# Tencent/PocketFlow

Hardware: NVIDIA H100
Metric: images_per_sec_compression_aware_training_step (higher is better)
Workload: dtype f32

## Files before the change

### pocketflow_b200/csrc/pf_conv_tma.cu

```cuda
#include <cuda.h>

#include "pf_conv_tc.cuh"
#include "pf_tma.cuh"

namespace pfconv {
using namespace pftma;

constexpr int kTmaMaxStages = 8;
constexpr int kTmaThreads = (kMmaWarps + 1) * 32;

struct TmaP {
  int M, Ng, BN, nk, n_tiles, total_tiles;
  int cblocks, R, S;
  int rows_hw, rows_w;
  int src_h, src_w;
  int base_w, base_h, str_w, str_h, flip;
  int na, nb;
  int accumulate, relu, ring, stage_budget;
  int chunked;
  FastDiv d_hw, d_w, d_ntiles, d_cblocks, d_s;
  EpiAff aff;
  const pf_tc_act_hdr* a_hdr;
  const float* csum;
  int nseg;
  pf_tc_bn_out bn;
};

constexpr int kPingPongWarps = 4;
constexpr int kPingPongThreads = (kMmaWarps + 4) * 32;
constexpr int kProducerRegs = 40, kConsumerRegs = 232;

__device__ __forceinline__ void conv_tma_epilogue_chunked(float (&acc)[2][64], const TmaP& p, float* acc_s,
                                                          int n0, long long off, long long* rowoff, float* out,
                                                          const float* bias, int wg, int q, int lane) {
  constexpr int P = acc_pitch(32);
  float* r0 = acc_s + (size_t)(16 * q + (lane >> 2)) * P + 2 * (lane & 3);
#pragma unroll
  for (int ch = 0; ch < 4; ++ch) {
    if (ch > 0) named_bar_sync(2 + wg, 128);
#pragma unroll
    for (int h = 0; h < 2; ++h)
#pragma unroll
      for (int jj = 0; jj < 4; ++jj) {
        const int j = 4 * ch + jj;
        *reinterpret_cast<float2*>(r0 + (size_t)(64 * h) * P + 8 * jj) = make_float2(acc[h][4 * j], acc[h][4 * j + 1]);
        *reinterpret_cast<float2*>(r0 + (size_t)(64 * h + 8) * P + 8 * jj) =
            make_float2(acc[h][4 * j + 2], acc[h][4 * j + 3]);
      }
    named_bar_sync(2 + wg, 128);
    epilogue_rows<0>(acc_s + (size_t)(32 * q) * P, 0, 32, off, rowoff, out, nullptr, bias, p.relu, n0 + 32 * ch, 32,
                     p.Ng, lane, nullptr, p.aff, 0.f, nullptr, nullptr, 0, p.bn);
  }
}

template <int AFF, int BN, int NA, int NB, bool BNO, bool U8>
__device__ __forceinline__ void conv_tma_consumer(const TmaP& p, uint8_t* smem, uint32_t stage_bytes,
                                                  uint32_t n_stages, uint64_t* full_bar, uint64_t* empty_bar,
                                                  uint64_t* ml_bar, uint64_t* epi_bar, int* tab_n0, float* out,
                                                  const float* bias, const float* residual) {
  const int tid = threadIdx.x, warp = tid >> 5, lane = tid & 31;
  const int wg = warp >> 2, q = warp & 3, wtid = tid & 127;
  constexpr uint32_t kRow = U8 ? 64u : 128u, kATile = TM * kRow;
  const uint32_t b_bytes = (uint32_t)BN * kRow;
  float* acc_s = reinterpret_cast<float*>(smem + p.stage_budget);
  long long* rowoff_all = reinterpret_cast<long long*>(acc_s + TM * acc_pitch(p.chunked ? 32 : BN));
  float* jrow_all = reinterpret_cast<float*>(rowoff_all + kMmaWarps * 32);
  float* aff_tab = jrow_all + kMmaWarps * 32;
  uint8_t* ring_all = reinterpret_cast<uint8_t*>(aff_tab + (AFF == 2 ? 2 * 256 : 0) + (BNO ? 4 * kMaxBN : 0));
  long long* rowoff = rowoff_all + warp * 32;
  float* jrow = jrow_all + warp * 32;
  uint8_t* ring = p.ring ? ring_all + (size_t)warp * p.ring * kRingSlotBytes : nullptr;
  const float* extra = residual ? residual : (p.accumulate ? out : nullptr);
  uint32_t it = (uint32_t)wg * (uint32_t)p.nk;
  for (int tile = blockIdx.x + wg * gridDim.x, j = 0; tile < p.total_tiles; tile += 2 * gridDim.x, ++j) {
    const bool wait_turn = wg == 1 || j > 0;
    const uint32_t turn_ph = (uint32_t)(wg == 1 ? j : j - 1) & 1u;
    if (wait_turn) mbar_wait_bounded(&ml_bar[wg], turn_ph);
    std::conditional_t<U8, int, float> acc[2][BN / 2];
#pragma unroll
    for (int h = 0; h < 2; ++h)
#pragma unroll
      for (int i = 0; i < BN / 2; ++i) acc[h][i] = 0;
    uint32_t s = it % n_stages, ph = (it / n_stages) & 1u, prev = 0;
    for (int ks = 0; ks < p.nk; ++ks) {
      mbar_wait_bounded(&full_bar[s], ph);
      const uint32_t a0 = smem_u32(smem + (size_t)s * stage_bytes), a1 = a0 + kATile;
      const uint32_t b0 = a0 + (uint32_t)NA * kATile, b1 = b0 + b_bytes;
      wgmma_fence();
      if constexpr (U8) {
#pragma unroll
        for (int kk = 0; kk < 2; ++kk) {
          const uint64_t db = make_smem_desc(b0 + kk * 32, 16, 512, kSwizzle64B);
#pragma unroll
          for (int h = 0; h < 2; ++h)
            WgmmaU8<BN>::mma(acc[h], make_smem_desc(a0 + (uint32_t)h * 64 * 64 + kk * 32, 16, 512, kSwizzle64B), db);
        }
      } else {
#pragma unroll
        for (int kk = 0; kk < BK / 16; ++kk) {
          const uint64_t db0 = make_smem_desc(b0 + kk * 32, 16, 1024), db1 = make_smem_desc(b1 + kk * 32, 16, 1024);
#pragma unroll
          for (int h = 0; h < 2; ++h) {
            const uint32_t ha = (uint32_t)h * 64 * 128 + kk * 32;
            wg_mma_kslice<BN, 0, NA, NB>(acc[h], make_smem_desc(a0 + ha, 16, 1024), make_smem_desc(a1 + ha, 16, 1024),
                                         db0, db1);
          }
        }
      }
      wgmma_commit();
      wgmma_wait<1>(acc);
      if (ks > 0) {
        __syncwarp();
        if (lane == 0) mbar_arrive(&empty_bar[prev]);
      }
      prev = s;
      if (++s == n_stages) { s = 0; ph ^= 1u; }
    }
    __syncwarp();
    if (lane == 0) mbar_arrive(&ml_bar[wg ^ 1]);
    wgmma_wait<0>(acc);
    if (p.nk > 0) {
      __syncwarp();
      if (lane == 0) mbar_arrive(&empty_bar[prev]);
    }
    it += 2u * (uint32_t)p.nk;
    const int mt = (int)fdiv((uint32_t)tile, p.d_ntiles);
    const int n0 = (tile - mt * p.n_tiles) * BN;
    const int m = mt * TM + q * 32 + lane;
    const long long off = m < p.M ? (long long)m * p.Ng : -1;
    float my_j = 0.f;
    if (AFF == 2 && p.csum && m < p.M) {
      const int img = (int)fdiv((uint32_t)m, p.d_hw);
      const int rem = m - img * p.rows_hw;
      const int y = (int)fdiv((uint32_t)rem, p.d_w), x = rem - y * p.rows_w;
      const int ow0 = p.base_w + x * p.str_w, oh0 = p.base_h + y * p.str_h;
      const int total = p.R * p.S * p.nseg;
      const float* cbase = p.csum + (size_t)img * p.src_h * p.src_w * p.nseg;
      auto term = [&](int u) -> float {
        if (u >= total) return 0.f;
        const int t = u / p.nseg, g = u - t * p.nseg;
        const int r = (int)fdiv((uint32_t)t, p.d_s), s_ = t - r * p.S;
        const int ih = oh0 + r, iw = ow0 + s_;
        const bool ok = (unsigned)ih < (unsigned)p.src_h && (unsigned)iw < (unsigned)p.src_w;
        return ok ? __ldg(cbase + ((size_t)ih * p.src_w + iw) * p.nseg + g) : 0.f;
      };
      float a0 = 0.f, a1 = 0.f, a2 = 0.f, a3 = 0.f;
      for (int u = 0; u < total; u += 4) {
        const float v0 = term(u), v1 = term(u + 1), v2 = term(u + 2), v3 = term(u + 3);
        a0 += v0; a1 += v1; a2 += v2; a3 += v3;
      }
      my_j = (a0 + a1) + (a2 + a3);
    }
    if (wait_turn) mbar_wait_bounded(&epi_bar[wg], turn_ph);
    constexpr bool TAB = AFF == 2 || BNO;
    if constexpr (BN == 128 && AFF == 0 && !BNO && !U8) {
      if (p.chunked) {
        conv_tma_epilogue_chunked(acc, p, acc_s, n0, off, rowoff, out, bias, wg, q, lane);
        __syncwarp();
        if (lane == 0) mbar_arrive(&epi_bar[wg ^ 1]);
        continue;
      }
    }
    wgmma_store_acc<BN>(acc[0], acc_s, acc_pitch(BN), 0, wtid);
    wgmma_store_acc<BN>(acc[1], acc_s, acc_pitch(BN), 64, wtid);
    const int tab_was = TAB ? *reinterpret_cast<volatile int*>(tab_n0) : 0;
    if (AFF == 2 && tab_was != n0) {
      float a_s = p.aff.a_scale ? __ldg(p.aff.a_scale) : 1.f;
      if (U8 && __ldg(&p.a_hdr->nplanes) != 1) a_s = __int_as_float(0x7fc00000);
      for (int c = wtid; c < BN; c += 128) {
        const bool cok = n0 + c < p.Ng;
        const int bi = p.aff.per_channel ? n0 + c : 0;
        const float al = cok ? __ldg(p.aff.w_alpha + bi) : 0.f, be = cok ? __ldg(p.aff.w_beta + bi) : 0.f;
        const float sx = al * p.aff.w_rk;
        aff_tab[c] = sx * a_s;
        aff_tab[256 + c] = fmaf(p.aff.w_centre, sx, be) * a_s;
      }
    }
    if (BNO && tab_was != n0) bn_table(p.bn, aff_tab + (AFF == 2 ? 512 : 0), n0, BN, p.Ng, wtid, 128);
    named_bar_sync(2 + wg, 128);
    if (TAB && tab_was != n0 && wtid == 0) *reinterpret_cast<volatile int*>(tab_n0) = n0;
    epilogue_rows<AFF, BNO>(acc_s + (size_t)(32 * q) * acc_pitch(BN), 0, 32, off, rowoff, out, extra, bias, p.relu, n0,
                            BN, p.Ng, lane, ring, p.aff, my_j, jrow, TAB ? aff_tab : nullptr, p.ring, p.bn);
    __syncwarp();
    if (lane == 0) mbar_arrive(&epi_bar[wg ^ 1]);
  }
}

template <int AFF, int BN, bool BNO = false, bool U8 = false>
__global__ void __launch_bounds__(kPingPongThreads, 1)
conv_tma_kernel(const __grid_constant__ CUtensorMap tmA0, const __grid_constant__ CUtensorMap tmA1,
                const __grid_constant__ CUtensorMap tmB0, const __grid_constant__ CUtensorMap tmB1,
                float* __restrict__ out, const float* __restrict__ bias, const float* __restrict__ residual,
                const __grid_constant__ TmaP p) {
  extern __shared__ uint8_t smem_raw[];
  uint8_t* smem = (uint8_t*)(((uintptr_t)smem_raw + 1023) & ~(uintptr_t)1023);
  __shared__ uint64_t full_bar[kTmaMaxStages], empty_bar[kTmaMaxStages], ml_bar[2], epi_bar[2];
  __shared__ int tab_n0;
  const int tid = threadIdx.x, warp = tid >> 5, lane = tid & 31;
  int na = p.na;
  if (p.a_hdr) na = (__ldg(&p.a_hdr->nplanes) == 2) ? 2 : 1;
  const int nb = p.nb;
  constexpr uint32_t kRow = U8 ? 64u : 128u, kATile = TM * kRow;
  const uint32_t b_bytes = (uint32_t)BN * kRow;
  const uint32_t stage_bytes = (uint32_t)na * kATile + (uint32_t)nb * b_bytes;
  const uint32_t n_stages = min((uint32_t)kTmaMaxStages, (uint32_t)p.stage_budget / stage_bytes);

  if (tid == 0) {
    for (int s = 0; s < kTmaMaxStages; ++s) {
      mbar_init(&full_bar[s], 1);
      mbar_init(&empty_bar[s], kPingPongWarps);
    }
    for (int w = 0; w < 2; ++w) {
      mbar_init(&ml_bar[w], kPingPongWarps);
      mbar_init(&epi_bar[w], kPingPongWarps);
    }
    tab_n0 = -1;
    fence_barrier_init();
  }
  __syncthreads();

  if (warp >= kMmaWarps) {
    setmaxnreg_dec<kProducerRegs>();
    if (warp == kMmaWarps && lane == 0) {
      prefetch_map(&tmA0);
      prefetch_map(&tmB0);
      if (na == 2) prefetch_map(&tmA1);
      if (nb == 2) prefetch_map(&tmB1);
      uint32_t s = 0, ph = 0;
      for (int tile = blockIdx.x; tile < p.total_tiles; tile += gridDim.x) {
        const int mt = (int)fdiv((uint32_t)tile, p.d_ntiles);
        const int n0 = (tile - mt * p.n_tiles) * BN;
        const int m0 = mt * TM;
        const int img = (int)fdiv((uint32_t)m0, p.d_hw);
        const int rem = m0 - img * p.rows_hw;
        const int y = (int)fdiv((uint32_t)rem, p.d_w), x = rem - y * p.rows_w;
        const int cw = p.base_w + x * p.str_w, ch = p.base_h + y * p.str_h;
        for (int ks = 0; ks < p.nk; ++ks) {
          mbar_wait_bounded(&empty_bar[s], ph ^ 1u);
          const int tap = (int)fdiv((uint32_t)ks, p.d_cblocks);
          const int cb = ks - tap * p.cblocks;
          const int r = (int)fdiv((uint32_t)tap, p.d_s), q = tap - r * p.S;
          const uint32_t ow = (uint32_t)(p.flip ? p.S - 1 - q : q), oh = (uint32_t)(p.flip ? p.R - 1 - r : r);
          const uint32_t sa = smem_u32(smem + (size_t)s * stage_bytes);
          const uint32_t sb = sa + (uint32_t)na * kATile;
          mbar_arrive_expect_tx(&full_bar[s], stage_bytes);
          load_im2col(sa, &tmA0, &full_bar[s], cb * BK, cw, ch, img, ow, oh);
          if (na == 2) load_im2col(sa + kATile, &tmA1, &full_bar[s], cb * BK, cw, ch, img, ow, oh);
          load_2d(sb, &tmB0, &full_bar[s], ks * BK, n0);
          if (nb == 2) load_2d(sb + b_bytes, &tmB1, &full_bar[s], ks * BK, n0);
          if (++s == n_stages) { s = 0; ph ^= 1u; }
        }
      }
    }
  } else {
    setmaxnreg_inc<kConsumerRegs>();
#define PF_TMA_CONSUMER(NA_, NB_)                                                                                    \
  conv_tma_consumer<AFF, BN, NA_, NB_, BNO, U8>(p, smem, stage_bytes, n_stages, full_bar, empty_bar, ml_bar, epi_bar, \
                                                &tab_n0, out, bias, residual)
    if constexpr (U8) {
      PF_TMA_CONSUMER(1, 1);
    } else {
      if (na == 2) {
        if (nb == 2) PF_TMA_CONSUMER(2, 2);
        else PF_TMA_CONSUMER(2, 1);
      } else {
        if (nb == 2) PF_TMA_CONSUMER(1, 2);
        else PF_TMA_CONSUMER(1, 1);
      }
    }
#undef PF_TMA_CONSUMER
  }
}

struct WgTmaP {
  TcGeom g;
  int Mtot, Npix, pps, splits, BN, n_tiles, tiles, total_units;
  int na, nb, stage_budget;
  FastDiv d_pq, d_q, d_c, d_s, d_tiles, d_ntiles;
  EpiAff aff;
  const pf_tc_act_hdr* x_hdr;
};
constexpr uint32_t kWgBlockBytes = BK * 128;

template <int AFF, int BN>
__global__ void __launch_bounds__(kTmaThreads, 1)
conv_tma_wgrad_kernel(const __grid_constant__ CUtensorMap tmX0, const __grid_constant__ CUtensorMap tmX1,
                      const __grid_constant__ CUtensorMap tmY0, const __grid_constant__ CUtensorMap tmY1,
                      float* __restrict__ partial, const __grid_constant__ WgTmaP p) {
  extern __shared__ uint8_t smem_raw[];
  uint8_t* smem = (uint8_t*)(((uintptr_t)smem_raw + 1023) & ~(uintptr_t)1023);
  __shared__ uint64_t full_bar[kTmaMaxStages], empty_bar[kTmaMaxStages];
  const int tid = threadIdx.x, warp = tid >> 5, lane = tid & 31;
  const TcGeom& g = p.g;
  const int nblkB = BN / 64;
  int na = p.na;
  if (p.x_hdr) na = (__ldg(&p.x_hdr->nplanes) == 2) ? 2 : 1;
  const int nb = p.nb;
  const uint32_t a_bytes = 2 * kWgBlockBytes, b_bytes = (uint32_t)nblkB * kWgBlockBytes;
  const uint32_t stage_bytes = (uint32_t)na * a_bytes + (uint32_t)nb * b_bytes;
  const uint32_t n_stages = min((uint32_t)kTmaMaxStages, (uint32_t)p.stage_budget / stage_bytes);
  float* acc_s = reinterpret_cast<float*>(smem + p.stage_budget);
  long long* rowoff_all = reinterpret_cast<long long*>(acc_s + TM * acc_pitch(BN));
  float* jrow_all = reinterpret_cast<float*>(rowoff_all + kMmaWarps * 32);
  if (tid == 0) {
    for (int s = 0; s < kTmaMaxStages; ++s) {
      mbar_init(&full_bar[s], 1);
      mbar_init(&empty_bar[s], kMmaWarps);
    }
    fence_barrier_init();
  }
  __syncthreads();
  struct Unit {
    int split, m0, n0, pbeg, nk;
  };
  auto decode = [&](int u) -> Unit {
    Unit r;
    r.split = (int)fdiv((uint32_t)u, p.d_tiles);
    const int t = u - r.split * p.tiles;
    const int mt = (int)fdiv((uint32_t)t, p.d_ntiles);
    r.m0 = mt * TM;
    r.n0 = (t - mt * p.n_tiles) * BN;
    r.pbeg = r.split * p.pps;
    const int pend = min(p.Npix, r.pbeg + p.pps);
    r.nk = (pend - r.pbeg + BK - 1) / BK;
    return r;
  };

  if (warp == kMmaWarps) {
    if (lane == 0) {
      prefetch_map(&tmX0);
      prefetch_map(&tmY0);
      if (na == 2) prefetch_map(&tmX1);
      if (nb == 2) prefetch_map(&tmY1);
      const int pq = g.P * g.Q;
      uint32_t s = 0, ph = 0;
      for (int u = blockIdx.x; u < p.total_units; u += gridDim.x) {
        const Unit un = decode(u);
        int c0[2], tr[2], tq[2], nvalid = 0;
#pragma unroll
        for (int b = 0; b < 2; ++b) {
          const int kf = un.m0 + 64 * b;
          const int tap = (int)fdiv((uint32_t)kf, p.d_c);
          c0[b] = kf - tap * g.C;
          tr[b] = (int)fdiv((uint32_t)tap, p.d_s);
          tq[b] = tap - tr[b] * g.S;
          if (kf < p.Mtot) nvalid = b + 1;
        }
        const uint32_t tx = (uint32_t)na * (uint32_t)nvalid * kWgBlockBytes + (uint32_t)nb * b_bytes;
        for (int ks = 0; ks < un.nk; ++ks) {
          mbar_wait_bounded(&empty_bar[s], ph ^ 1u);
          const int pix0 = un.pbeg + ks * BK;
          const int pn = (int)fdiv((uint32_t)pix0, p.d_pq);
          const int rem = pix0 - pn * pq;
          const int oh = (int)fdiv((uint32_t)rem, p.d_q), ow = rem - oh * g.Q;
          const int cw = ow * g.sw - g.pl, ch = oh * g.sh - g.pt;
          const uint32_t sa = smem_u32(smem + (size_t)s * stage_bytes);
          const uint32_t sb = sa + (uint32_t)na * a_bytes;
          mbar_arrive_expect_tx(&full_bar[s], tx);
          for (int b = 0; b < nvalid; ++b) {
            load_im2col(sa + b * kWgBlockBytes, &tmX0, &full_bar[s], c0[b], cw, ch, pn, (uint32_t)tq[b], (uint32_t)tr[b]);
            if (na == 2)
              load_im2col(sa + a_bytes + b * kWgBlockBytes, &tmX1, &full_bar[s], c0[b], cw, ch, pn, (uint32_t)tq[b],
                          (uint32_t)tr[b]);
          }
          for (int j = 0; j < nblkB; ++j) {
            load_2d(sb + j * kWgBlockBytes, &tmY0, &full_bar[s], un.n0 + 64 * j, pix0);
            if (nb == 2) load_2d(sb + b_bytes + j * kWgBlockBytes, &tmY1, &full_bar[s], un.n0 + 64 * j, pix0);
          }
          if (++s == n_stages) { s = 0; ph ^= 1u; }
        }
      }
    }
  } else {
    const int wg = warp >> 2, q = warp & 3;
    long long* rowoff = rowoff_all + warp * 32;
    float* jrow = jrow_all + warp * 32;
    auto consume = [&](auto na_c, auto nb_c) {
    constexpr int NA = decltype(na_c)::value, NB = decltype(nb_c)::value;
    uint32_t s = 0, ph = 0;
    for (int u = blockIdx.x; u < p.total_units; u += gridDim.x) {
      const Unit un = decode(u);
      float acc[BN / 2];
#pragma unroll
      for (int i = 0; i < BN / 2; ++i) acc[i] = 0.f;
      uint32_t prev = 0;
      for (int ks = 0; ks < un.nk; ++ks) {
        mbar_wait_bounded(&full_bar[s], ph);
        const uint32_t base = smem_u32(smem + (size_t)s * stage_bytes);
        const uint32_t a0 = base + (uint32_t)wg * kWgBlockBytes, a1 = a0 + a_bytes;
        const uint32_t b0 = base + (uint32_t)NA * a_bytes, b1 = b0 + b_bytes;
        wg_mma_stage<BN, 1, NA, NB>(acc, a0, a1, b0, b1, 2048, 2048, kWgBlockBytes, 1024, kWgBlockBytes, 1024);
        wgmma_wait<1>(acc);
        if (ks > 0) {
          __syncwarp();
          if (lane == 0) mbar_arrive(&empty_bar[prev]);
        }
        prev = s;
        if (++s == n_stages) { s = 0; ph ^= 1u; }
      }
      wgmma_wait<0>(acc);
      if (un.nk > 0) {
        __syncwarp();
        if (lane == 0) mbar_arrive(&empty_bar[prev]);
      }
      const int em = un.m0 + q * 32 + lane;
      const long long off = em < p.Mtot ? ((long long)un.split * p.Mtot + em) * g.K : -1;
      wg_tile_to_smem<BN>(acc, acc_s, tid);
      epilogue_tile_a<AFF>(acc_s, warp, off, rowoff, partial, nullptr, nullptr, 0, un.n0, BN, g.K, lane, nullptr, p.aff,
                           0.f, jrow, pf_tc_bn_out{});
    }
    };
    using one = std::integral_constant<int, 1>;
    using two = std::integral_constant<int, 2>;
    if (na == 2) {
      if (nb == 2) consume(two(), two());
      else consume(two(), one());
    } else {
      if (nb == 2) consume(one(), two());
      else consume(one(), one());
    }
  }
}

static int g_feed_override = -1;
void conv_tma_set_feed(int mode) { g_feed_override = mode < 0 ? -1 : (mode ? 1 : 0); }
static bool tma_enabled() {
  if (g_feed_override >= 0) return g_feed_override == 1;
  static int on = -1;
  if (on < 0) {
    const char* v = getenv("PF_TC_FEED");
    on = !(v && strcmp(v, "lsu") == 0);
  }
  return on == 1;
}

bool conv_tma_eligible(int pass, const TcGeom& g) {
  if (!tma_enabled()) return false;
  if (pass == 0) return g.C % 64 == 0 && g.K % 16 == 0 && g.sh <= 8 && g.sw <= 8 && g.R <= 16 && g.S <= 16;
  if (pass == 1) return g.K % 64 == 0 && g.C % 16 == 0 && g.sh == 1 && g.sw == 1 && g.R <= 16 && g.S <= 16;
  return g.C % 64 == 0 && g.K % 64 == 0 && g.sh <= 8 && g.sw <= 8;
}

bool conv_tma_u8_eligible(const TcGeom& g) {
  return g.C % 64 == 0 && g.K % 64 == 0 && g.sh <= 8 && g.sw <= 8 && g.R <= 16 && g.S <= 16;
}

static int pick_bn(int Ng) {
  int BN = Ng >= 128 ? 128 : (Ng >= 64 ? 64 : (Ng >= 32 ? 32 : 16));
  const int forced = env_int("PF_TC_BN", 0);
  if (forced >= 16 && forced <= kMaxBN && forced <= ((Ng + 15) / 16) * 16 && (forced & (forced - 1)) == 0) BN = forced;
  return BN;
}

#define PF_TMA_ENCODE(call, who)                                                               \
  do {                                                                                         \
    const int e__ = (call);                                                                    \
    if (e__ != 0) {                                                                            \
      pf_set_error("%s: tensor-map encoding failed (%d): %s", who, e__, #call);                \
      return PF_ERR_INVALID_ARG;                                                               \
    }                                                                                          \
  } while (0)

int conv_tma_launch(int pass, const TcGeom& g, const pf_tc_act& a, const pf_tc_wt& w, float* out, int accumulate,
                    const float* bias, int relu, const float* residual, cudaStream_t st, const char* who,
                    const pf_tc_bn_out* bn, bool u8) {
  TmaP p;
  memset(&p, 0, sizeof(p));
  const int CC = pass == 0 ? g.C : g.K;
  const int Hs = pass == 0 ? g.H : g.P, Ws = pass == 0 ? g.W : g.Q;
  const int Ho = pass == 0 ? g.P : g.H, Wo = pass == 0 ? g.Q : g.W;
  const int64_t M64 = (int64_t)g.N * Ho * Wo;
  PF_REQUIRE(M64 < (1ll << 31), "%s: too many rows", who);
  p.M = (int)M64;
  p.Ng = pass == 0 ? g.K : g.C;
  const int Kdim = g.R * g.S * CC;
  p.nk = Kdim / BK;
  p.cblocks = CC / BK;
  p.R = g.R;
  p.S = g.S;
  p.rows_hw = Ho * Wo;
  p.rows_w = Wo;
  p.src_h = Hs;
  p.src_w = Ws;
  if (pass == 0) {
    p.base_w = -g.pl; p.base_h = -g.pt; p.str_w = g.sw; p.str_h = g.sh; p.flip = 0;
  } else {
    p.base_w = g.pl - (g.S - 1); p.base_h = g.pt - (g.R - 1); p.str_w = 1; p.str_h = 1; p.flip = 1;
  }
  p.accumulate = accumulate;
  p.relu = relu;
  const int m_tiles = (p.M + TM - 1) / TM;
  const int BN = u8 ? (p.Ng >= 128 ? 128 : 64) : pick_bn(p.Ng);
  p.BN = BN;
  p.n_tiles = (p.Ng + BN - 1) / BN;
  p.total_tiles = m_tiles * p.n_tiles;
  p.d_hw = make_fastdiv((uint32_t)p.rows_hw);
  p.d_w = make_fastdiv((uint32_t)p.rows_w);
  p.d_ntiles = make_fastdiv((uint32_t)p.n_tiles);
  p.d_cblocks = make_fastdiv((uint32_t)p.cblocks);
  p.d_s = make_fastdiv((uint32_t)g.S);
  p.na = a.plane1 ? 2 : 1;
  p.nb = w.plane1 ? 2 : 1;
  p.a_hdr = a.hdr;
  PF_REQUIRE(a.hdr == nullptr || a.plane1 != nullptr || u8, "%s: an operand with a device header needs both planes",
             who);
  int aff = 0;
  PF_REQUIRE(!u8 || (pass == 0 && w.alpha != nullptr && a.hdr != nullptr && a.plane1 == nullptr && w.plane1 == nullptr &&
                      p.Ng % 64 == 0),
             "%s: u8 operands are a forward pass of activation levels with a header and weight levels", who);
  if (w.alpha) {
    PF_REQUIRE(w.beta != nullptr && w.bits >= 1 && w.bits <= 8, "%s: weight levels need alpha, beta and 1..8 bits", who);
    PF_REQUIRE(a.csum != nullptr && a.nseg >= 1, "%s: weight levels need the operand's channel sums", who);
    aff = 2;
    p.aff.w_alpha = w.alpha;
    p.aff.w_beta = w.beta;
    p.aff.per_channel = w.per_channel;
    p.aff.w_rk = 1.f / (float)((1 << w.bits) - 1);
    p.aff.w_centre = u8 ? 0.f : (float)(1 << (w.bits - 1));
    p.aff.a_scale = a.hdr ? &a.hdr->scale : nullptr;
    p.csum = a.csum;
    p.nseg = a.nseg;
  } else if (a.hdr) {
    aff = 1;
    p.aff.a_scale = &a.hdr->scale;
  }
  PF_REQUIRE(bn == nullptr || (pass == 0 && (aff == 0 || u8)), "%s: the folded batch norm needs a split-bf16 or u8 forward",
             who);
  if (bn) p.bn = *bn;
  const int row_bytes = u8 ? 64 : 128;
  const int stage_max = (p.na * TM + p.nb * BN) * row_bytes;
  const bool has_extra = residual != nullptr || accumulate;
  const int aff_tab_bytes = (aff == 2 ? 2 * 256 * 4 : 0) + (bn ? 4 * kMaxBN * 4 : 0);
  const int epi_bytes = epi_fixed_bytes(BN) + aff_tab_bytes;
  int budget = (kSmemLimit - epi_bytes) / 1024 * 1024;
  int ring_bytes = 0;
  p.ring = 0;
  if (has_extra && env_int("PF_TC_RING", 1) && BN >= 64) {
    const int need = std::min(3, p.nk + 1);
    for (int depth = kRingDepth; depth >= 2 && !p.ring; depth >>= 1) {
      const int rb = kMmaWarps * depth * kRingSlotBytes;
      if ((budget - rb) / stage_max >= need) {
        p.ring = depth;
        ring_bytes = rb;
      }
    }
    if (p.ring) budget = (kSmemLimit - epi_bytes - ring_bytes) / 1024 * 1024;
  }
  int used_epi = epi_bytes;
  p.chunked = 0;
  if (BN == 128 && aff == 0 && !bn && !has_extra && p.nk >= 3) {
    const int chunk_epi = epi_fixed_bytes(32);
    const int chunk_budget = (kSmemLimit - chunk_epi) / 1024 * 1024;
    if (budget / stage_max < 3 && chunk_budget / stage_max > budget / stage_max) {
      p.chunked = 1;
      budget = chunk_budget;
      used_epi = chunk_epi;
    }
  }
  PF_REQUIRE(budget / stage_max >= 2 || p.nk <= 1, "%s: shared-memory plan failed (BN %d)", who, BN);
  p.stage_budget = budget;
  const size_t smem = (size_t)budget + used_epi + (p.ring ? ring_bytes : 0);
  const int grid = std::min(p.total_tiles, PF_NUM_SMS);
  record_plan(pf_tc_plan{0, 1, pass, 0, BN, aff, p.na, p.nb, 0, p.ring, 0, budget, p.total_tiles, grid, 0, 0});
  if (p.total_tiles == 0) return PF_OK;
  alignas(64) CUtensorMap tA0, tA1, tB0, tB1;
  const int Kpad = pad64(Kdim);
  if (u8) {
    PF_TMA_ENCODE(encode_im2col_u8(&tA0, a.plane0, g.N, Hs, Ws, CC, p.base_w, p.base_h, Wo, Ho, p.str_w, p.str_h, BK, TM), who);
    PF_TMA_ENCODE(encode_2d_u8(&tB0, w.plane0, (uint64_t)Kpad, (uint64_t)p.Ng, (uint64_t)Kpad, BK, (uint32_t)BN), who);
    auto kern = BN == 128 ? (bn ? conv_tma_kernel<2, 128, true, true> : conv_tma_kernel<2, 128, false, true>)
                          : (bn ? conv_tma_kernel<2, 64, true, true> : conv_tma_kernel<2, 64, false, true>);
    PF_CUDA(cudaFuncSetAttribute(kern, cudaFuncAttributeMaxDynamicSharedMemorySize, (int)smem));
    kern<<<grid, kPingPongThreads, smem, st>>>(tA0, tA0, tB0, tB0, out, bias, residual, p);
    PF_CHECK_LAUNCH(who);
    return PF_OK;
  }
  PF_TMA_ENCODE(encode_im2col_bf16(&tA0, a.plane0, g.N, Hs, Ws, CC, p.base_w, p.base_h, Wo, Ho, p.str_w, p.str_h, BK, TM), who);
  if (a.plane1)
    PF_TMA_ENCODE(encode_im2col_bf16(&tA1, a.plane1, g.N, Hs, Ws, CC, p.base_w, p.base_h, Wo, Ho, p.str_w, p.str_h, BK, TM), who);
  else
    tA1 = tA0;
  PF_TMA_ENCODE(encode_2d_bf16(&tB0, w.plane0, (uint64_t)Kpad, (uint64_t)p.Ng, (uint64_t)Kpad, BK, (uint32_t)BN), who);
  if (w.plane1)
    PF_TMA_ENCODE(encode_2d_bf16(&tB1, w.plane1, (uint64_t)Kpad, (uint64_t)p.Ng, (uint64_t)Kpad, BK, (uint32_t)BN), who);
  else
    tB1 = tB0;
  cudaError_t err = cudaSuccess;
  with_bn(BN, [&](auto bn_c) {
    constexpr int B = decltype(bn_c)::value;
    auto kern = bn ? conv_tma_kernel<0, B, true>
                   : (aff == 2 ? conv_tma_kernel<2, B> : (aff == 1 ? conv_tma_kernel<1, B> : conv_tma_kernel<0, B>));
    err = cudaFuncSetAttribute(kern, cudaFuncAttributeMaxDynamicSharedMemorySize, (int)smem);
    if (err == cudaSuccess) kern<<<grid, kPingPongThreads, smem, st>>>(tA0, tA1, tB0, tB1, out, bias, residual, p);
  });
  PF_CUDA(err);
  PF_CHECK_LAUNCH(who);
  return PF_OK;
}

int conv_tma_wgrad_launch(const TcGeom& g, const pf_tc_act& x, const pf_tc_act& dy, int BN, int pps, int splits,
                          float* partial, cudaStream_t st, const char* who) {
  WgTmaP p;
  memset(&p, 0, sizeof(p));
  p.g = g;
  p.Mtot = g.R * g.S * g.C;
  p.Npix = g.N * g.P * g.Q;
  p.BN = BN;
  p.pps = pps;
  p.splits = splits;
  const int m_tiles = (p.Mtot + TM - 1) / TM;
  p.n_tiles = (g.K + BN - 1) / BN;
  p.tiles = m_tiles * p.n_tiles;
  p.total_units = p.tiles * p.splits;
  p.d_pq = make_fastdiv((uint32_t)(g.P * g.Q));
  p.d_q = make_fastdiv((uint32_t)g.Q);
  p.d_c = make_fastdiv((uint32_t)g.C);
  p.d_s = make_fastdiv((uint32_t)g.S);
  p.d_tiles = make_fastdiv((uint32_t)p.tiles);
  p.d_ntiles = make_fastdiv((uint32_t)p.n_tiles);
  p.na = x.plane1 ? 2 : 1;
  p.nb = dy.plane1 ? 2 : 1;
  p.x_hdr = x.hdr;
  PF_REQUIRE(x.hdr == nullptr || x.plane1 != nullptr, "%s: an operand with a device header needs both planes", who);
  PF_REQUIRE(dy.hdr == nullptr, "%s: the gradient operand is always split-bf16", who);
  int aff = 0;
  if (x.hdr) {
    aff = 1;
    p.aff.a_scale = &x.hdr->scale;
  }
  const int stage_max = p.na * 2 * (int)kWgBlockBytes + p.nb * (BN / 64) * (int)kWgBlockBytes;
  const int budget = (kSmemLimit - epi_fixed_bytes(BN)) / 1024 * 1024;
  PF_REQUIRE(budget / stage_max >= 2, "%s: shared-memory plan failed (BN %d)", who, BN);
  p.stage_budget = budget;
  const size_t smem = (size_t)budget + epi_fixed_bytes(BN);
  const int grid = std::min(p.total_units, PF_NUM_SMS);
  record_plan(pf_tc_plan{0, 1, 2, 0, BN, aff, p.na, p.nb, 0, 0, 0, budget, p.total_units, grid, splits, pps});
  if (p.total_units == 0) return PF_OK;
  alignas(64) CUtensorMap tX0, tX1, tY0, tY1;
  PF_TMA_ENCODE(encode_im2col_bf16(&tX0, x.plane0, g.N, g.H, g.W, g.C, -g.pl, -g.pt, g.Q, g.P, g.sw, g.sh, BK, BK), who);
  if (x.plane1)
    PF_TMA_ENCODE(encode_im2col_bf16(&tX1, x.plane1, g.N, g.H, g.W, g.C, -g.pl, -g.pt, g.Q, g.P, g.sw, g.sh, BK, BK), who);
  else
    tX1 = tX0;
  PF_TMA_ENCODE(encode_2d_bf16(&tY0, dy.plane0, (uint64_t)g.K, (uint64_t)p.Npix, (uint64_t)g.K, BK, BK), who);
  if (dy.plane1)
    PF_TMA_ENCODE(encode_2d_bf16(&tY1, dy.plane1, (uint64_t)g.K, (uint64_t)p.Npix, (uint64_t)g.K, BK, BK), who);
  else
    tY1 = tY0;
  auto kern = BN == 128 ? (aff == 1 ? conv_tma_wgrad_kernel<1, 128> : conv_tma_wgrad_kernel<0, 128>)
                        : (aff == 1 ? conv_tma_wgrad_kernel<1, 64> : conv_tma_wgrad_kernel<0, 64>);
  PF_CUDA(cudaFuncSetAttribute(kern, cudaFuncAttributeMaxDynamicSharedMemorySize, (int)smem));
  kern<<<grid, kTmaThreads, smem, st>>>(tX0, tX1, tY0, tY1, partial, p);
  PF_CHECK_LAUNCH(who);
  return PF_OK;
}

}
```

### pocketflow_b200/csrc/pf_tma.cuh

```cuda
#pragma once
#include <cuda.h>
#include <cuda_runtime.h>
#include <stdint.h>

#include "pf_tc_common.cuh"

namespace pftma {

typedef CUresult (*EncodeTiledFn)(CUtensorMap*, CUtensorMapDataType, cuuint32_t, void*, const cuuint64_t*,
                                  const cuuint64_t*, const cuuint32_t*, const cuuint32_t*, CUtensorMapInterleave,
                                  CUtensorMapSwizzle, CUtensorMapL2promotion, CUtensorMapFloatOOBfill);
typedef CUresult (*EncodeIm2colFn)(CUtensorMap*, CUtensorMapDataType, cuuint32_t, void*, const cuuint64_t*,
                                   const cuuint64_t*, const int*, const int*, cuuint32_t, cuuint32_t, const cuuint32_t*,
                                   CUtensorMapInterleave, CUtensorMapSwizzle, CUtensorMapL2promotion,
                                   CUtensorMapFloatOOBfill);

inline void* driver_entry(const char* name) {
  void* fn = nullptr;
  cudaDriverEntryPointQueryResult qres;
  if (cudaGetDriverEntryPoint(name, &fn, cudaEnableDefault, &qres) != cudaSuccess || qres != cudaDriverEntryPointSuccess)
    return nullptr;
  return fn;
}

inline void small_tensor_fixup(CUtensorMap* m, uint64_t tensor_bytes) {
  static int drv = -1;
  if (drv < 0) cudaDriverGetVersion(&drv);
  if (drv <= 13010 && tensor_bytes < 131072) reinterpret_cast<uint64_t*>(m)[1] &= ~(1ull << 21);
}

inline int encode_2d(CUtensorMap* m, CUtensorMapDataType dtype, uint32_t esize, CUtensorMapSwizzle swizzle,
                     const void* base, uint64_t cols, uint64_t rows, uint64_t pitch_elems, uint32_t box_cols,
                     uint32_t box_rows) {
  static EncodeTiledFn fn = (EncodeTiledFn)driver_entry("cuTensorMapEncodeTiled");
  if (!fn) return -1;
  const cuuint64_t dims[2] = {cols, rows};
  const cuuint64_t strides[1] = {pitch_elems * esize};
  const cuuint32_t box[2] = {box_cols, box_rows};
  const cuuint32_t estr[2] = {1, 1};
  const CUresult r = fn(m, dtype, 2, const_cast<void*>(base), dims, strides, box, estr, CU_TENSOR_MAP_INTERLEAVE_NONE,
                        swizzle, CU_TENSOR_MAP_L2_PROMOTION_L2_256B, CU_TENSOR_MAP_FLOAT_OOB_FILL_NONE);
  if (r != CUDA_SUCCESS) return (int)r;
  small_tensor_fixup(m, rows * pitch_elems * esize);
  return 0;
}
inline int encode_2d_bf16(CUtensorMap* m, const void* base, uint64_t cols, uint64_t rows, uint64_t pitch_elems,
                          uint32_t box_cols, uint32_t box_rows) {
  return encode_2d(m, CU_TENSOR_MAP_DATA_TYPE_BFLOAT16, 2, CU_TENSOR_MAP_SWIZZLE_128B, base, cols, rows, pitch_elems,
                   box_cols, box_rows);
}
inline int encode_2d_u8(CUtensorMap* m, const void* base, uint64_t cols, uint64_t rows, uint64_t pitch_elems,
                        uint32_t box_cols, uint32_t box_rows) {
  return encode_2d(m, CU_TENSOR_MAP_DATA_TYPE_UINT8, 1, CU_TENSOR_MAP_SWIZZLE_64B, base, cols, rows, pitch_elems,
                   box_cols, box_rows);
}

inline int encode_im2col(CUtensorMap* m, CUtensorMapDataType dtype, uint32_t esize, CUtensorMapSwizzle swizzle,
                         const void* base, int n, int h, int w, int c, int base_w, int base_h, int out_w, int out_h,
                         int str_w, int str_h, uint32_t channels, uint32_t pixels) {
  static EncodeIm2colFn fn = (EncodeIm2colFn)driver_entry("cuTensorMapEncodeIm2col");
  if (!fn) return -1;
  const cuuint64_t dims[4] = {(cuuint64_t)c, (cuuint64_t)w, (cuuint64_t)h, (cuuint64_t)n};
  const cuuint64_t strides[3] = {(cuuint64_t)c * esize, (cuuint64_t)w * c * esize, (cuuint64_t)h * w * c * esize};
  const int lower[2] = {base_w, base_h};
  const int upper[2] = {(out_w - 1) * str_w + base_w + 1 - w, (out_h - 1) * str_h + base_h + 1 - h};
  if (lower[0] < -128 || lower[0] > 127 || lower[1] < -128 || lower[1] > 127 || upper[0] < -128 || upper[0] > 127 ||
      upper[1] < -128 || upper[1] > 127 || str_w > 8 || str_h > 8)
    return -2;
  const cuuint32_t estr[4] = {1, (cuuint32_t)str_w, (cuuint32_t)str_h, 1};
  const CUresult r = fn(m, dtype, 4, const_cast<void*>(base), dims, strides, lower, upper, channels, pixels, estr,
                        CU_TENSOR_MAP_INTERLEAVE_NONE, swizzle, CU_TENSOR_MAP_L2_PROMOTION_L2_256B,
                        CU_TENSOR_MAP_FLOAT_OOB_FILL_NONE);
  if (r != CUDA_SUCCESS) return (int)r;
  small_tensor_fixup(m, (uint64_t)n * h * w * c * esize);
  return 0;
}
inline int encode_im2col_bf16(CUtensorMap* m, const void* base, int n, int h, int w, int c, int base_w, int base_h,
                              int out_w, int out_h, int str_w, int str_h, uint32_t channels, uint32_t pixels) {
  return encode_im2col(m, CU_TENSOR_MAP_DATA_TYPE_BFLOAT16, 2, CU_TENSOR_MAP_SWIZZLE_128B, base, n, h, w, c, base_w,
                       base_h, out_w, out_h, str_w, str_h, channels, pixels);
}
inline int encode_im2col_u8(CUtensorMap* m, const void* base, int n, int h, int w, int c, int base_w, int base_h,
                            int out_w, int out_h, int str_w, int str_h, uint32_t channels, uint32_t pixels) {
  return encode_im2col(m, CU_TENSOR_MAP_DATA_TYPE_UINT8, 1, CU_TENSOR_MAP_SWIZZLE_64B, base, n, h, w, c, base_w,
                       base_h, out_w, out_h, str_w, str_h, channels, pixels);
}

#ifdef __CUDACC__
__device__ __forceinline__ void prefetch_map(const CUtensorMap* m) {
  asm volatile("prefetch.tensormap [%0];" ::"l"(reinterpret_cast<uint64_t>(m)) : "memory");
}
__device__ __forceinline__ void mbar_arrive_expect_tx(uint64_t* bar, uint32_t bytes) {
  asm volatile("mbarrier.arrive.expect_tx.shared::cta.b64 _, [%0], %1;" ::"r"(pftc::smem_u32(bar)), "r"(bytes) : "memory");
}
__device__ __forceinline__ void load_2d(uint32_t dst, const CUtensorMap* m, uint64_t* bar, int col, int row) {
  asm volatile(
      "cp.async.bulk.tensor.2d.shared::cluster.global.tile.mbarrier::complete_tx::bytes [%0], [%1, {%3, %4}], [%2];" ::"r"(dst),
      "l"(reinterpret_cast<uint64_t>(m)), "r"(pftc::smem_u32(bar)), "r"(col), "r"(row)
      : "memory");
}
__device__ __forceinline__ void load_im2col(uint32_t dst, const CUtensorMap* m, uint64_t* bar, int c, int w, int h, int n,
                                            uint32_t off_w, uint32_t off_h) {
  asm volatile(
      "cp.async.bulk.tensor.4d.shared::cluster.global.im2col.mbarrier::complete_tx::bytes [%0], [%1, {%3, %4, %5, %6}], [%2], "
      "{%7, %8};" ::"r"(dst),
      "l"(reinterpret_cast<uint64_t>(m)), "r"(pftc::smem_u32(bar)), "r"(c), "r"(w), "r"(h), "r"(n), "h"((uint16_t)off_w),
      "h"((uint16_t)off_h)
      : "memory");
}
#endif

}
```

Measured before the change: 2770.

## Extend chunked conv epilogue to fused BN-output path with per-warpgroup tables

```diff
diff --git a/pocketflow_b200/csrc/pf_conv_tma.cu b/pocketflow_b200/csrc/pf_conv_tma.cu
--- a/pocketflow_b200/csrc/pf_conv_tma.cu
+++ b/pocketflow_b200/csrc/pf_conv_tma.cu
@@ -30,11 +30,46 @@
 constexpr int kPingPongThreads = (kMmaWarps + 4) * 32;
 constexpr int kProducerRegs = 40, kConsumerRegs = 232;
 
+__device__ __forceinline__ void conv_tma_chunk_bn_rows(const float* acc, const long long* rowoff, float* out,
+                                                       const float* bias, int relu, int n0, int Ng, int lane,
+                                                       const float* bt, const pf_tc_bn_out& bn) {
+  constexpr int P = acc_pitch(32);
+  const int cv = (lane & 7) * 4, rsub = lane >> 3;
+  if (n0 + cv + 3 >= Ng) return;
+  const float* a = acc + (size_t)rsub * P + cv;
+#pragma unroll 2
+  for (int u = 0; u < 8; ++u) {
+    const long long o = rowoff[4 * u + rsub];
+    if (o < 0) continue;
+    const size_t e = (size_t)o + n0 + cv;
+    float4 w = *reinterpret_cast<const float4*>(a + (size_t)(4 * u) * P);
+    if (bias) {
+      const float4 bb = __ldg(reinterpret_cast<const float4*>(bias + n0 + cv));
+      w.x = __fadd_rn(w.x, bb.x); w.y = __fadd_rn(w.y, bb.y); w.z = __fadd_rn(w.z, bb.z); w.w = __fadd_rn(w.w, bb.w);
+    }
+    if (relu) { w.x = fmaxf(w.x, 0.f); w.y = fmaxf(w.y, 0.f); w.z = fmaxf(w.z, 0.f); w.w = fmaxf(w.w, 0.f); }
+    __stcs(reinterpret_cast<float4*>(out + e), w);
+    const float4 brs = *reinterpret_cast<const float4*>(bt + cv), bmu = *reinterpret_cast<const float4*>(bt + 32 + cv);
+    const float4 bga = *reinterpret_cast<const float4*>(bt + 64 + cv), bbe = *reinterpret_cast<const float4*>(bt + 96 + cv);
+    const int act = bn.act;
+    w.x = pf_bn_act(w.x, bmu.x, brs.x, bga.x, bbe.x, act); w.y = pf_bn_act(w.y, bmu.y, brs.y, bga.y, bbe.y, act);
+    w.z = pf_bn_act(w.z, bmu.z, brs.z, bga.z, bbe.z, act); w.w = pf_bn_act(w.w, bmu.w, brs.w, bga.w, bbe.w, act);
+    if (bn.y) *reinterpret_cast<float4*>(bn.y + e) = w;
+    if (bn.hi) pf_st_planes4(bn.hi, bn.lo, (int64_t)e, w);
+  }
+}
+
+template <bool BNO>
 __device__ __forceinline__ void conv_tma_epilogue_chunked(float (&acc)[2][64], const TmaP& p, float* acc_s,
                                                           int n0, long long off, long long* rowoff, float* out,
-                                                          const float* bias, int wg, int q, int lane) {
+                                                          const float* bias, const float* bn_tab, int wg, int q,
+                                                          int lane) {
   constexpr int P = acc_pitch(32);
   float* r0 = acc_s + (size_t)(16 * q + (lane >> 2)) * P + 2 * (lane & 3);
+  if (BNO) {
+    rowoff[lane] = off;
+    __syncwarp();
+  }
 #pragma unroll
   for (int ch = 0; ch < 4; ++ch) {
     if (ch > 0) named_bar_sync(2 + wg, 128);
@@ -48,9 +83,14 @@
             make_float2(acc[h][4 * j + 2], acc[h][4 * j + 3]);
       }
     named_bar_sync(2 + wg, 128);
-    epilogue_rows<0>(acc_s + (size_t)(32 * q) * P, 0, 32, off, rowoff, out, nullptr, bias, p.relu, n0 + 32 * ch, 32,
-                     p.Ng, lane, nullptr, p.aff, 0.f, nullptr, nullptr, 0, p.bn);
-  }
+    if (BNO)
+      conv_tma_chunk_bn_rows(acc_s + (size_t)(32 * q) * P, rowoff, out, bias, p.relu, n0 + 32 * ch, p.Ng, lane,
+                             bn_tab + 128 * ch, p.bn);
+    else
+      epilogue_rows<0>(acc_s + (size_t)(32 * q) * P, 0, 32, off, rowoff, out, nullptr, bias, p.relu, n0 + 32 * ch, 32,
+                       p.Ng, lane, nullptr, p.aff, 0.f, nullptr, nullptr, 0, p.bn);
+  }
+  if (BNO) __syncwarp();
 }
 
 template <int AFF, int BN, int NA, int NB, bool BNO, bool U8>
@@ -75,6 +115,14 @@
   for (int tile = blockIdx.x + wg * gridDim.x, j = 0; tile < p.total_tiles; tile += 2 * gridDim.x, ++j) {
     const bool wait_turn = wg == 1 || j > 0;
     const uint32_t turn_ph = (uint32_t)(wg == 1 ? j : j - 1) & 1u;
+    if constexpr (BN == 128 && AFF == 0 && BNO && !U8) {
+      auto col0 = [&](int t) { return (t - (int)fdiv((uint32_t)t, p.d_ntiles) * p.n_tiles) * BN; };
+      const int tn0 = col0(tile);
+      if (p.chunked && (j == 0 || tn0 != col0(tile - 2 * (int)gridDim.x))) {
+        if (j > 0) named_bar_sync(2 + wg, 128);
+        bn_table(p.bn, aff_tab + 4 * kMaxBN * wg + 128 * q, tn0 + 32 * q, 32, p.Ng, lane, 32);
+      }
+    }
     if (wait_turn) mbar_wait_bounded(&ml_bar[wg], turn_ph);
     std::conditional_t<U8, int, float> acc[2][BN / 2];
 #pragma unroll
@@ -153,9 +201,10 @@
     }
     if (wait_turn) mbar_wait_bounded(&epi_bar[wg], turn_ph);
     constexpr bool TAB = AFF == 2 || BNO;
-    if constexpr (BN == 128 && AFF == 0 && !BNO && !U8) {
+    if constexpr (BN == 128 && AFF == 0 && !U8) {
       if (p.chunked) {
-        conv_tma_epilogue_chunked(acc, p, acc_s, n0, off, rowoff, out, bias, wg, q, lane);
+        conv_tma_epilogue_chunked<BNO>(acc, p, acc_s, n0, off, rowoff, out, bias, aff_tab + 4 * kMaxBN * wg, wg, q,
+                                       lane);
         __syncwarp();
         if (lane == 0) mbar_arrive(&epi_bar[wg ^ 1]);
         continue;
@@ -548,8 +597,8 @@
   }
   int used_epi = epi_bytes;
   p.chunked = 0;
-  if (BN == 128 && aff == 0 && !bn && !has_extra && p.nk >= 3) {
-    const int chunk_epi = epi_fixed_bytes(32);
+  if (BN == 128 && aff == 0 && !has_extra && p.nk >= 3) {
+    const int chunk_epi = epi_fixed_bytes(32) + 2 * aff_tab_bytes;
     const int chunk_budget = (kSmemLimit - chunk_epi) / 1024 * 1024;
     if (budget / stage_max < 3 && chunk_budget / stage_max > budget / stage_max) {
       p.chunked = 1;
```

Measured after the change: 2842, median of 6. 2.6% higher.

## Halve TMA K-stage depth to fit more pipeline stages for two-plane BN128 conv

Applied to the files above, without the earlier changes.

```diff
diff --git a/pocketflow_b200/csrc/pf_conv_tma.cu b/pocketflow_b200/csrc/pf_conv_tma.cu
--- a/pocketflow_b200/csrc/pf_conv_tma.cu
+++ b/pocketflow_b200/csrc/pf_conv_tma.cu
@@ -53,14 +53,18 @@
   }
 }
 
-template <int AFF, int BN, int NA, int NB, bool BNO, bool U8>
+template <bool U8, int KC>
+__host__ __device__ constexpr uint32_t tma_row_bytes() { return U8 ? 64u : 2u * KC; }
+
+template <int AFF, int BN, int NA, int NB, bool BNO, bool U8, int KC>
 __device__ __forceinline__ void conv_tma_consumer(const TmaP& p, uint8_t* smem, uint32_t stage_bytes,
                                                   uint32_t n_stages, uint64_t* full_bar, uint64_t* empty_bar,
                                                   uint64_t* ml_bar, uint64_t* epi_bar, int* tab_n0, float* out,
                                                   const float* bias, const float* residual) {
   const int tid = threadIdx.x, warp = tid >> 5, lane = tid & 31;
   const int wg = warp >> 2, q = warp & 3, wtid = tid & 127;
-  constexpr uint32_t kRow = U8 ? 64u : 128u, kATile = TM * kRow;
+  constexpr uint32_t kRow = tma_row_bytes<U8, KC>(), kATile = TM * kRow;
+  constexpr uint32_t kSbo = 8 * kRow, kSw = kRow == 128u ? kSwizzle128B : kSwizzle64B;
   const uint32_t b_bytes = (uint32_t)BN * kRow;
   float* acc_s = reinterpret_cast<float*>(smem + p.stage_budget);
   long long* rowoff_all = reinterpret_cast<long long*>(acc_s + TM * acc_pitch(p.chunked ? 32 : BN));
@@ -97,13 +101,13 @@
         }
       } else {
 #pragma unroll
-        for (int kk = 0; kk < BK / 16; ++kk) {
-          const uint64_t db0 = make_smem_desc(b0 + kk * 32, 16, 1024), db1 = make_smem_desc(b1 + kk * 32, 16, 1024);
+        for (int kk = 0; kk < KC / 16; ++kk) {
+          const uint64_t db0 = make_smem_desc(b0 + kk * 32, 16, kSbo, kSw), db1 = make_smem_desc(b1 + kk * 32, 16, kSbo, kSw);
 #pragma unroll
           for (int h = 0; h < 2; ++h) {
-            const uint32_t ha = (uint32_t)h * 64 * 128 + kk * 32;
-            wg_mma_kslice<BN, 0, NA, NB>(acc[h], make_smem_desc(a0 + ha, 16, 1024), make_smem_desc(a1 + ha, 16, 1024),
-                                         db0, db1);
+            const uint32_t ha = (uint32_t)h * 64 * kRow + kk * 32;
+            wg_mma_kslice<BN, 0, NA, NB>(acc[h], make_smem_desc(a0 + ha, 16, kSbo, kSw),
+                                         make_smem_desc(a1 + ha, 16, kSbo, kSw), db0, db1);
           }
         }
       }
@@ -186,7 +190,7 @@
   }
 }
 
-template <int AFF, int BN, bool BNO = false, bool U8 = false>
+template <int AFF, int BN, bool BNO = false, bool U8 = false, int KC = BK>
 __global__ void __launch_bounds__(kPingPongThreads, 1)
 conv_tma_kernel(const __grid_constant__ CUtensorMap tmA0, const __grid_constant__ CUtensorMap tmA1,
                 const __grid_constant__ CUtensorMap tmB0, const __grid_constant__ CUtensorMap tmB1,
@@ -200,7 +204,8 @@
   int na = p.na;
   if (p.a_hdr) na = (__ldg(&p.a_hdr->nplanes) == 2) ? 2 : 1;
   const int nb = p.nb;
-  constexpr uint32_t kRow = U8 ? 64u : 128u, kATile = TM * kRow;
+  constexpr uint32_t kRow = tma_row_bytes<U8, KC>(), kATile = TM * kRow;
+  constexpr int kStageC = U8 ? BK : KC;
   const uint32_t b_bytes = (uint32_t)BN * kRow;
   const uint32_t stage_bytes = (uint32_t)na * kATile + (uint32_t)nb * b_bytes;
   const uint32_t n_stages = min((uint32_t)kTmaMaxStages, (uint32_t)p.stage_budget / stage_bytes);
@@ -244,10 +249,10 @@
           const uint32_t sa = smem_u32(smem + (size_t)s * stage_bytes);
           const uint32_t sb = sa + (uint32_t)na * kATile;
           mbar_arrive_expect_tx(&full_bar[s], stage_bytes);
-          load_im2col(sa, &tmA0, &full_bar[s], cb * BK, cw, ch, img, ow, oh);
-          if (na == 2) load_im2col(sa + kATile, &tmA1, &full_bar[s], cb * BK, cw, ch, img, ow, oh);
-          load_2d(sb, &tmB0, &full_bar[s], ks * BK, n0);
-          if (nb == 2) load_2d(sb + b_bytes, &tmB1, &full_bar[s], ks * BK, n0);
+          load_im2col(sa, &tmA0, &full_bar[s], cb * kStageC, cw, ch, img, ow, oh);
+          if (na == 2) load_im2col(sa + kATile, &tmA1, &full_bar[s], cb * kStageC, cw, ch, img, ow, oh);
+          load_2d(sb, &tmB0, &full_bar[s], ks * kStageC, n0);
+          if (nb == 2) load_2d(sb + b_bytes, &tmB1, &full_bar[s], ks * kStageC, n0);
           if (++s == n_stages) { s = 0; ph ^= 1u; }
         }
       }
@@ -255,8 +260,8 @@
   } else {
     setmaxnreg_inc<kConsumerRegs>();
 #define PF_TMA_CONSUMER(NA_, NB_)                                                                                    \
-  conv_tma_consumer<AFF, BN, NA_, NB_, BNO, U8>(p, smem, stage_bytes, n_stages, full_bar, empty_bar, ml_bar, epi_bar, \
-                                                &tab_n0, out, bias, residual)
+  conv_tma_consumer<AFF, BN, NA_, NB_, BNO, U8, KC>(p, smem, stage_bytes, n_stages, full_bar, empty_bar, ml_bar,     \
+                                                    epi_bar, &tab_n0, out, bias, residual)
     if constexpr (U8) {
       PF_TMA_CONSUMER(1, 1);
     } else {
@@ -559,6 +564,13 @@
   }
   PF_REQUIRE(budget / stage_max >= 2 || p.nk <= 1, "%s: shared-memory plan failed (BN %d)", who, BN);
   p.stage_budget = budget;
+  const bool kc32 = !u8 && BN == 128 && p.na == 2 && p.nb == 2 && budget / stage_max < 3 &&
+                    env_int("PF_TC_KSTAGE", 32) != 64;
+  if (kc32) {
+    p.nk *= 2;
+    p.cblocks *= 2;
+    p.d_cblocks = make_fastdiv((uint32_t)p.cblocks);
+  }
   const size_t smem = (size_t)budget + used_epi + (p.ring ? ring_bytes : 0);
   const int grid = std::min(p.total_tiles, PF_NUM_SMS);
   record_plan(pf_tc_plan{0, 1, pass, 0, BN, aff, p.na, p.nb, 0, p.ring, 0, budget, p.total_tiles, grid, 0, 0});
@@ -572,6 +584,25 @@
                           : (bn ? conv_tma_kernel<2, 64, true, true> : conv_tma_kernel<2, 64, false, true>);
     PF_CUDA(cudaFuncSetAttribute(kern, cudaFuncAttributeMaxDynamicSharedMemorySize, (int)smem));
     kern<<<grid, kPingPongThreads, smem, st>>>(tA0, tA0, tB0, tB0, out, bias, residual, p);
+    PF_CHECK_LAUNCH(who);
+    return PF_OK;
+  }
+  if (kc32) {
+    constexpr int KC = BK / 2;
+    PF_TMA_ENCODE(encode_im2col_bf16_sw64(&tA0, a.plane0, g.N, Hs, Ws, CC, p.base_w, p.base_h, Wo, Ho, p.str_w, p.str_h,
+                                          KC, TM), who);
+    PF_TMA_ENCODE(encode_im2col_bf16_sw64(&tA1, a.plane1, g.N, Hs, Ws, CC, p.base_w, p.base_h, Wo, Ho, p.str_w, p.str_h,
+                                          KC, TM), who);
+    PF_TMA_ENCODE(encode_2d_bf16_sw64(&tB0, w.plane0, (uint64_t)Kpad, (uint64_t)p.Ng, (uint64_t)Kpad, KC, (uint32_t)BN),
+                  who);
+    PF_TMA_ENCODE(encode_2d_bf16_sw64(&tB1, w.plane1, (uint64_t)Kpad, (uint64_t)p.Ng, (uint64_t)Kpad, KC, (uint32_t)BN),
+                  who);
+    auto kern = bn ? conv_tma_kernel<0, 128, true, false, KC>
+                   : (aff == 2 ? conv_tma_kernel<2, 128, false, false, KC>
+                               : (aff == 1 ? conv_tma_kernel<1, 128, false, false, KC>
+                                           : conv_tma_kernel<0, 128, false, false, KC>));
+    PF_CUDA(cudaFuncSetAttribute(kern, cudaFuncAttributeMaxDynamicSharedMemorySize, (int)smem));
+    kern<<<grid, kPingPongThreads, smem, st>>>(tA0, tA1, tB0, tB1, out, bias, residual, p);
     PF_CHECK_LAUNCH(who);
     return PF_OK;
   }
diff --git a/pocketflow_b200/csrc/pf_tma.cuh b/pocketflow_b200/csrc/pf_tma.cuh
--- a/pocketflow_b200/csrc/pf_tma.cuh
+++ b/pocketflow_b200/csrc/pf_tma.cuh
@@ -49,6 +49,11 @@
   return encode_2d(m, CU_TENSOR_MAP_DATA_TYPE_BFLOAT16, 2, CU_TENSOR_MAP_SWIZZLE_128B, base, cols, rows, pitch_elems,
                    box_cols, box_rows);
 }
+inline int encode_2d_bf16_sw64(CUtensorMap* m, const void* base, uint64_t cols, uint64_t rows, uint64_t pitch_elems,
+                               uint32_t box_cols, uint32_t box_rows) {
+  return encode_2d(m, CU_TENSOR_MAP_DATA_TYPE_BFLOAT16, 2, CU_TENSOR_MAP_SWIZZLE_64B, base, cols, rows, pitch_elems,
+                   box_cols, box_rows);
+}
 inline int encode_2d_u8(CUtensorMap* m, const void* base, uint64_t cols, uint64_t rows, uint64_t pitch_elems,
                         uint32_t box_cols, uint32_t box_rows) {
   return encode_2d(m, CU_TENSOR_MAP_DATA_TYPE_UINT8, 1, CU_TENSOR_MAP_SWIZZLE_64B, base, cols, rows, pitch_elems,
@@ -78,6 +83,11 @@
 inline int encode_im2col_bf16(CUtensorMap* m, const void* base, int n, int h, int w, int c, int base_w, int base_h,
                               int out_w, int out_h, int str_w, int str_h, uint32_t channels, uint32_t pixels) {
   return encode_im2col(m, CU_TENSOR_MAP_DATA_TYPE_BFLOAT16, 2, CU_TENSOR_MAP_SWIZZLE_128B, base, n, h, w, c, base_w,
+                       base_h, out_w, out_h, str_w, str_h, channels, pixels);
+}
+inline int encode_im2col_bf16_sw64(CUtensorMap* m, const void* base, int n, int h, int w, int c, int base_w, int base_h,
+                                   int out_w, int out_h, int str_w, int str_h, uint32_t channels, uint32_t pixels) {
+  return encode_im2col(m, CU_TENSOR_MAP_DATA_TYPE_BFLOAT16, 2, CU_TENSOR_MAP_SWIZZLE_64B, base, n, h, w, c, base_w,
                        base_h, out_w, out_h, str_w, str_h, channels, pixels);
 }
 inline int encode_im2col_u8(CUtensorMap* m, const void* base, int n, int h, int w, int c, int base_w, int base_h,
```

Measured after the change: 2772 before, 2828 after (median of 6 runs). 1.02x the previous value.

## Extend chunked low-smem epilogue to fused BN-output convolutions

Applied to the files above, without the earlier changes.

```diff
diff --git a/pocketflow_b200/csrc/pf_conv_tma.cu b/pocketflow_b200/csrc/pf_conv_tma.cu
--- a/pocketflow_b200/csrc/pf_conv_tma.cu
+++ b/pocketflow_b200/csrc/pf_conv_tma.cu
@@ -30,9 +30,11 @@
 constexpr int kPingPongThreads = (kMmaWarps + 4) * 32;
 constexpr int kProducerRegs = 40, kConsumerRegs = 232;
 
+template <bool BNO>
 __device__ __forceinline__ void conv_tma_epilogue_chunked(float (&acc)[2][64], const TmaP& p, float* acc_s,
                                                           int n0, long long off, long long* rowoff, float* out,
-                                                          const float* bias, int wg, int q, int lane) {
+                                                          const float* bias, const float* tab,
+                                                          int wg, int q, int lane) {
   constexpr int P = acc_pitch(32);
   float* r0 = acc_s + (size_t)(16 * q + (lane >> 2)) * P + 2 * (lane & 3);
 #pragma unroll
@@ -50,6 +52,34 @@
     named_bar_sync(2 + wg, 128);
     epilogue_rows<0>(acc_s + (size_t)(32 * q) * P, 0, 32, off, rowoff, out, nullptr, bias, p.relu, n0 + 32 * ch, 32,
                      p.Ng, lane, nullptr, p.aff, 0.f, nullptr, nullptr, 0, p.bn);
+  }
+  if (BNO) {
+    const int cv = (lane & 7) * 4;
+    int ro[8];
+#pragma unroll
+    for (int u = 0; u < 8; ++u) {
+      const long long o = __shfl_sync(0xffffffffu, off, 4 * u + (lane >> 3));
+      ro[u] = o < 0 ? -1 : (int)(o >> 2);
+    }
+    __syncwarp();
+    const pf_tc_bn_out& bn = p.bn;
+#pragma unroll 1
+    for (int c = cv; c < 128; c += 32) {
+      if (n0 + c + 3 >= p.Ng) continue;
+      const float4 brs = *reinterpret_cast<const float4*>(tab + c), bmu = *reinterpret_cast<const float4*>(tab + 128 + c);
+      const float4 bga = *reinterpret_cast<const float4*>(tab + 256 + c);
+      const float4 bbe = *reinterpret_cast<const float4*>(tab + 384 + c);
+#pragma unroll
+      for (int u = 0; u < 8; ++u) {
+        if (ro[u] < 0) continue;
+        const int64_t e = ((int64_t)ro[u] << 2) + n0 + c;
+        float4 w = *reinterpret_cast<const float4*>(out + e);
+        w.x = pf_bn_act(w.x, bmu.x, brs.x, bga.x, bbe.x, bn.act); w.y = pf_bn_act(w.y, bmu.y, brs.y, bga.y, bbe.y, bn.act);
+        w.z = pf_bn_act(w.z, bmu.z, brs.z, bga.z, bbe.z, bn.act); w.w = pf_bn_act(w.w, bmu.w, brs.w, bga.w, bbe.w, bn.act);
+        if (bn.y) *reinterpret_cast<float4*>(bn.y + e) = w;
+        if (bn.hi) pf_st_planes4(bn.hi, bn.lo, e, w);
+      }
+    }
   }
 }
 
@@ -71,10 +101,21 @@
   float* jrow = jrow_all + warp * 32;
   uint8_t* ring = p.ring ? ring_all + (size_t)warp * p.ring * kRingSlotBytes : nullptr;
   const float* extra = residual ? residual : (p.accumulate ? out : nullptr);
+  constexpr bool CHUNK_BNO = BN == 128 && AFF == 0 && BNO && !U8;
+  float* wg_tab = aff_tab + wg * 4 * kMaxBN;
+  int wg_tab_n0 = -1;
   uint32_t it = (uint32_t)wg * (uint32_t)p.nk;
   for (int tile = blockIdx.x + wg * gridDim.x, j = 0; tile < p.total_tiles; tile += 2 * gridDim.x, ++j) {
     const bool wait_turn = wg == 1 || j > 0;
     const uint32_t turn_ph = (uint32_t)(wg == 1 ? j : j - 1) & 1u;
+    if (CHUNK_BNO && p.chunked) {
+      const int n0 = (tile - (int)fdiv((uint32_t)tile, p.d_ntiles) * p.n_tiles) * BN;
+      if (n0 != wg_tab_n0) {
+        named_bar_sync(2 + wg, 128);
+        bn_table(p.bn, wg_tab, n0, BN, p.Ng, wtid, 128);
+        wg_tab_n0 = n0;
+      }
+    }
     if (wait_turn) mbar_wait_bounded(&ml_bar[wg], turn_ph);
     std::conditional_t<U8, int, float> acc[2][BN / 2];
 #pragma unroll
@@ -153,9 +194,9 @@
     }
     if (wait_turn) mbar_wait_bounded(&epi_bar[wg], turn_ph);
     constexpr bool TAB = AFF == 2 || BNO;
-    if constexpr (BN == 128 && AFF == 0 && !BNO && !U8) {
+    if constexpr (BN == 128 && AFF == 0 && !U8) {
       if (p.chunked) {
-        conv_tma_epilogue_chunked(acc, p, acc_s, n0, off, rowoff, out, bias, wg, q, lane);
+        conv_tma_epilogue_chunked<BNO>(acc, p, acc_s, n0, off, rowoff, out, bias, wg_tab, wg, q, lane);
         __syncwarp();
         if (lane == 0) mbar_arrive(&epi_bar[wg ^ 1]);
         continue;
@@ -548,8 +589,8 @@
   }
   int used_epi = epi_bytes;
   p.chunked = 0;
-  if (BN == 128 && aff == 0 && !bn && !has_extra && p.nk >= 3) {
-    const int chunk_epi = epi_fixed_bytes(32);
+  if (BN == 128 && aff == 0 && !has_extra && p.nk >= (bn ? 16 : 3)) {
+    const int chunk_epi = epi_fixed_bytes(32) + 2 * aff_tab_bytes;
     const int chunk_budget = (kSmemLimit - chunk_epi) / 1024 * 1024;
     if (budget / stage_max < 3 && chunk_budget / stage_max > budget / stage_max) {
       p.chunked = 1;
```

Result: faster. 2768 before, 2811 after, median of 6 (+1.6%).
